# yjcaimeow/pointnerf

Measured on AMD Instinct MI355X. Metric: Mray-samples/sec at 800x800, K=8, 2M neural points; PSNR delta vs ref, higher is better.
Workload: dtype fp32h2

## Files before the change

### pointnerf_amd/csrc/aggregate_x3.hip

```cpp
#include "agg_common.h"


namespace pnr {
namespace {

constexpr int kXT = 64;
constexpr int kXTS = kXT / kKN;
constexpr int kHidPlane = 32 * 64 * 16;
constexpr int kHidTile = 2 * kHidPlane;
constexpr int kXG = 34;
constexpr int kPG = 8;
constexpr int kPlaneX = kXG * kXT * 16;
constexpr int kPlaneP = kPG * kXT * 16;
constexpr int kP1Pitch = kHid + 4;

template <bool H>
struct XL {
  static constexpr int NPL = H ? 2 : 3;
  static constexpr int NPW = H ? 2 : 3;
  static constexpr unsigned kOne = H ? 0x3C00u : 0x3F80u;
  static constexpr int OffPE = NPL * kPlaneX;
  static constexpr int OffEx = OffPE + NPL * kPlaneP;
  static constexpr int NWB = H ? 3 : 2;
  static constexpr int OffWt = OffEx + 2 * 8 * kXT * 4;
  static constexpr int OffPr = OffWt + NWB * kXT * 4;
  static constexpr int OffSf = OffPr + 2 * kXT * 4;
  static constexpr int OffAp = OffSf + NWB * kXTS * 4;
  static constexpr int OffWa = OffAp + 4 * kXT * 4;
  static constexpr int OffH4 = OffWa + kHid * 4;
  static constexpr int OffTq = OffH4 + (H ? kXT * kP1Pitch * 4 : 0);
  static constexpr size_t Lds = (size_t)OffTq + 16;
  static_assert(OffSf % 16 == 0 && OffWa % 16 == 0 && OffH4 % 16 == 0, "16-B aligned LDS arrays");
  static_assert(kXT * kP1Pitch * 4 <= NPL * kPlaneX, "parked P1 fits the layer-input area");
  static_assert(Lds <= 160 * 1024, "LDS budget");
};

constexpr int kProducerPrio = 3;
constexpr int kStoreWindowPrio = 0;

typedef float f32x2n __attribute__((ext_vector_type(2)));
typedef float f32x4n __attribute__((ext_vector_type(4)));

struct X3Args {
  pnr_points pts;
  pnr_samples s;
  pnr_mlp w;
  SplitW wx;
  const float* p1;
  float* hid;
  int32_t* vmask;
  float* out_feat;
  float* out_weight;
  float* out_conf;
  int32_t* tile_ctr;
  pnr_agg_saved sv;
};

__device__ __forceinline__ bool xcd_mode(int64_t nt) { return nt >= 2 * (int64_t)gridDim.x + 16; }
__device__ __forceinline__ int64_t xcd_lo(int64_t nt, int x) { return nt * x / 8; }
__device__ __forceinline__ int64_t xcd_nb(int x) { return ((int)gridDim.x - x + 7) / 8; }

__device__ __forceinline__ int64_t first_tile(int64_t nt) {
  if (!xcd_mode(nt)) return blockIdx.x;
  return xcd_lo(nt, blockIdx.x & 7) + (blockIdx.x >> 3);
}

__device__ __forceinline__ int64_t take_tile(const X3Args& A, int64_t nt) {
  if (!xcd_mode(nt)) return (int64_t)gridDim.x + atomicAdd(A.tile_ctr, 1);
  const int x0 = blockIdx.x & 7;
  for (int i = 0; i < 8; ++i) {
    const int x = (x0 + i) & 7;
    const int64_t t = xcd_lo(nt, x) + xcd_nb(x) + atomicAdd(A.tile_ctr + x, 1);
    if (t < xcd_lo(nt, x + 1)) return t;
  }
  return nt;
}

__device__ __forceinline__ __amdgpu_buffer_rsrc_t rsrc(const void* base) {
  return __builtin_amdgcn_make_buffer_rsrc(const_cast<void*>(base), 0, 0x7fffffff, 0x00020000);
}

template <bool H, int NTK = 8>
__device__ __forceinline__ void load_w(uint4 (&a)[2][XL<H>::NPW], __amdgpu_buffer_rsrc_t rs, int voff, int t) {
  constexpr int NPW = XL<H>::NPW;
#pragma unroll
  for (int T = 0; T < 2; ++T)
#pragma unroll
    for (int pl = 0; pl < NPW; ++pl)
      a[T][pl] = __builtin_bit_cast(
          uint4, __builtin_amdgcn_raw_buffer_load_b128(
                     rs, voff + pl * 1024, (t * NTK + T) * NPW * 1024, 0));
}

template <bool H>
struct WRing {
  static constexpr int kWD = 3;
  uint4 a[kWD][2][XL<H>::NPW];
};

template <bool H, int NTK = 8>
__device__ __forceinline__ void prime(WRing<H>& w, __amdgpu_buffer_rsrc_t rs, int voff) {
#pragma unroll
  for (int d = 0; d < WRing<H>::kWD; ++d) load_w<H, NTK>(w.a[d], rs, voff, d);
}

template <bool H, int NTK = 8, bool ACC2 = false, bool ZACC = false>
__device__ __forceinline__ void layer(f32x16 (&acc)[4], f32x16 (&corr)[4], WRing<H>& w, __amdgpu_buffer_rsrc_t rs,
                                      int voff, const char* planes, int pstride, int nsteps, int lane) {
  static_assert(ACC2 || !ZACC, "zero-start accumulators: with two accumulator sets only");
  static_assert(H || !ACC2, "two accumulator sets: the f16 split only");
  constexpr int NPL = XL<H>::NPL, NPW = XL<H>::NPW, kWD = WRing<H>::kWD;
  const int c = lane & 31, h = lane >> 5;
  const char* base = planes + (h * kXT + c) * 16;
  auto ldb = [&](int t, int pt, uint4 (&bb)[NPL]) {
#pragma unroll
    for (int pl = 0; pl < NPL; ++pl)
      bb[pl] = *reinterpret_cast<const uint4*>(base + pl * pstride + (2 * t * kXT + 32 * pt) * 16);
// ... 146 lines not shown
          lrelu_splith(v[0], v[1], k, ks, a0, a1);
          lrelu_splith(v[2], v[3], k, ks, b0, b1);
          char* d = planes + ((4 * (T0 + T) + q) * kXT + 32 * pt + c) * 16 + 8 * h;
          *reinterpret_cast<uint2*>(d) = make_uint2(a0, b0);
          *reinterpret_cast<uint2*>(d + pstride) = make_uint2(a1, b1);
        }
    return;
  }
#pragma unroll
  for (int pt = 0; pt < 2; ++pt)
#pragma unroll
    for (int T = 0; T < 2; ++T)
#pragma unroll
      for (int q = 0; q < 4; ++q) {
        const f32x16& v = acc[2 * pt + T];
        unsigned a0, a1, a2, b0, b1, b2;
        split2(fmaxf(v[4 * q], s * v[4 * q]), fmaxf(v[4 * q + 1], s * v[4 * q + 1]), a0, a1, a2);
        split2(fmaxf(v[4 * q + 2], s * v[4 * q + 2]), fmaxf(v[4 * q + 3], s * v[4 * q + 3]), b0, b1, b2);
        char* d = planes + ((4 * (T0 + T) + q) * kXT + 32 * pt + c) * 16 + 8 * h;
        *reinterpret_cast<uint2*>(d) = make_uint2(a0, b0);
        *reinterpret_cast<uint2*>(d + kPlaneX) = make_uint2(a1, b1);
        *reinterpret_cast<uint2*>(d + 2 * kPlaneX) = make_uint2(a2, b2);
      }
}

template <bool H>
__device__ __forceinline__ void store_act(const f32x16 (&acc)[4], char* planes, float s, float mul, int lane,
                                          int T0, int pstride = kPlaneX) {
  store_act<H, false>(acc, acc, planes, s, mul, lane, T0, pstride);
}

template <bool H>
__device__ __forceinline__ void acc_init(f32x16 (&acc)[4], const float* bias, float inv_scale, int lane, int T0) {
  if constexpr (H) {
    const int h = lane >> 5;
#pragma unroll
    for (int T = 0; T < 2; ++T)
#pragma unroll
      for (int q = 0; q < 4; ++q) {
        const float4 b = *reinterpret_cast<const float4*>(bias + 32 * (T0 + T) + 8 * q + 4 * h);
        const float v[4] = {b.x * inv_scale, b.y * inv_scale, b.z * inv_scale, b.w * inv_scale};
#pragma unroll
        for (int i = 0; i < 4; ++i) {
          acc[T][4 * q + i] = v[i];
          acc[2 + T][4 * q + i] = v[i];
        }
      }
  } else {
#pragma unroll
    for (int i = 0; i < 4; ++i) acc[i] = (f32x16){0.f};
  }
}
constexpr int kBiasSteps(bool H) { return H ? 16 : 17; }

template <bool H>
__device__ __forceinline__ void store_group(char* planes, int pstride, int g, int pair, const float (&v)[8]) {
  if constexpr (H) {
    uint4 p0, p1;
    splith(v[0], v[1], p0.x, p1.x);
    splith(v[2], v[3], p0.y, p1.y);
    splith(v[4], v[5], p0.z, p1.z);
    splith(v[6], v[7], p0.w, p1.w);
    char* d = planes + (g * kXT + pair) * 16;
    *reinterpret_cast<uint4*>(d) = p0;
    *reinterpret_cast<uint4*>(d + pstride) = p1;
    return;
  }
  uint4 p0, p1, p2;
  split2(v[0], v[1], p0.x, p1.x, p2.x);
  split2(v[2], v[3], p0.y, p1.y, p2.y);
  split2(v[4], v[5], p0.z, p1.z, p2.z);
  split2(v[6], v[7], p0.w, p1.w, p2.w);
  char* d = planes + (g * kXT + pair) * 16;
  *reinterpret_cast<uint4*>(d) = p0;
  *reinterpret_cast<uint4*>(d + pstride) = p1;
  *reinterpret_cast<uint4*>(d + 2 * pstride) = p2;
}

struct GatherState {
  int64_t tile;
  int64_t row;
  int pid;
  float sw[3], sp[3];
  int64_t dmap;
  bool active;
};

__device__ __forceinline__ void gather_row(const X3Args& A, int64_t tile, int lane, GatherState& g) {
  const int64_t v = tile * kXTS + (lane >> 3);
  g.tile = tile;
  g.active = v < eff_n(A.s);
  g.row = g.active ? sample_row(A.s, v) : 0;
}

__device__ __forceinline__ void gather_sample(const X3Args& A, int lane, GatherState& g) {
  const int k = lane & 7, K = A.s.K;
  g.pid = (g.active && k < K) ? A.s.pidx[g.row * K + k] : -1;
#pragma unroll
  for (int a = 0; a < 3; ++a) {
    g.sw[a] = g.active ? A.s.sample_w[g.row * 3 + a] : 0.f;
    g.sp[a] = g.active ? A.s.sample_p[g.row * 3 + a] : 0.f;
  }
  g.dmap = A.s.dir_map ? (int64_t)A.s.dir_map[g.row] : g.row;
}

template <bool H, bool TR = false>
__device__ __forceinline__ void gather(const X3Args& A, const GatherState& g, int nb, int nw, char* lds, int pw, int lane,
                                       float (&dr6)[6]) {
  using L = XL<H>;
  float Rw[9];
#pragma unroll
  for (int i = 0; i < 9; ++i) Rw[i] = A.w.rw2c ? A.w.rw2c[i] : (i % 4 == 0 ? 1.f : 0.f);
  float cam_c[3] = {0.f, 0.f, 0.f}, cam_R[9] = {1.f, 0.f, 0.f, 0.f, 1.f, 0.f, 0.f, 0.f, 1.f};
  if (!A.pts.pers) {
#pragma unroll
    for (int i = 0; i < 3; ++i) cam_c[i] = A.pts.campos[i];
#pragma unroll
    for (int i = 0; i < 9; ++i) cam_R[i] = A.pts.camrot[i];
  }
  const int j = lane >> 3, k = lane & 7;
  const int K = A.s.K;
  const bool active = g.active;
  const int64_t row = g.row;
  const bool valid = g.pid >= 0;
  const int64_t prow = valid ? g.pid : (active && k < K ? 0 : -1);
  float sw[3], sp[3], vd[3] = {0.f, 0.f, 0.f};
#pragma unroll
  for (int a = 0; a < 3; ++a) {
    sw[a] = g.sw[a];
    sp[a] = g.sp[a];
  }
  const int64_t drow = active ? g.dmap / A.s.dir_div : 0;
  if (active && pw == 0) {
#pragma unroll
    for (int a = 0; a < 3; ++a) vd[a] = A.s.dirs[drow * 3 + a];
  }
  float pw3[3] = {0.f, 0.f, 0.f}, pp[3] = {0.f, 0.f, 0.f}, col[3] = {0.f, 0.f, 0.f}, pdir[3] = {0.f, 0.f, 0.f};
  float cf = 1.f;
  if (valid) {
#pragma unroll
    for (int a = 0; a < 3; ++a) pw3[a] = A.pts.xyz[prow * 3 + a];
    if (pw == 0) {
#pragma unroll
      for (int a = 0; a < 3; ++a) {
        col[a] = A.pts.color ? A.pts.color[prow * 3 + a] : 0.f;
        pdir[a] = A.pts.dir ? A.pts.dir[prow * 3 + a] : 0.f;
      }
    }
    if (A.pts.pers) {
#pragma unroll
      for (int a = 0; a < 3; ++a) pp[a] = A.pts.pers[prow * 3 + a];
    } else {
      pair_pers(A.pts, A.s, drow, pw3, cam_c, cam_R, pp);
    }
  }
  if (pw == 0 && A.pts.conf && prow >= 0) cf = A.pts.conf[prow];
  float d6[6];
  d6[0] = pw3[0] - sw[0];
  d6[1] = pw3[1] - sw[1];
  d6[2] = pw3[2] - sw[2];
  d6[3] = pp[0] * pp[2] - sp[0] * sp[2];
  d6[4] = pp[1] * pp[2] - sp[1] * sp[2];
  d6[5] = pp[2] - sp[2];
  mat3(Rw, d6, dr6);
  dr6[3] = d6[3];
  dr6[4] = d6[4];
  dr6[5] = d6[5];
  if (A.pts.rw2c) rot_point(A.pts.rw2c, prow, d6, dr6);
  if (pw == 0) {
    const float nrm = sqrtf(d6[0] * d6[0] + d6[1] * d6[1] + d6[2] * d6[2]);
    const float wl = valid ? 1.f / fmaxf(nrm, 1e-6f) : 0.f;
    const float wsum = xor8_sum(wl);
    const float wn = wl / fmaxf(wsum, 1e-8f);
    const float confc = fminf(fmaxf(cf, 1e-4f), 1.f);
    const bool samp_valid = xor8_sum(valid ? 1.f : 0.f) > 0.f;
    float vrot[3], drot[3];
    mat3(Rw, vd, vrot);
    mat3(Rw, pdir, drot);
    if (A.pts.rw2c) {
      rot_point(A.pts.rw2c, prow, pdir, drot);
      rot_point(A.pts.rw2c, active ? slot0_point(A.s, row) : 0, vd, vrot);
    }
    const float dot = drot[0] * vrot[0] + drot[1] * vrot[1] + drot[2] * vrot[2];
    const float ex[8] = {col[0], col[1], col[2], drot[0] - vrot[0], drot[1] - vrot[1], drot[2] - vrot[2], dot, 1.f};
    float* exL = reinterpret_cast<float*>(lds + L::OffEx) + nb * 8 * kXT;
#pragma unroll
    for (int e = 0; e < 8; ++e) exL[e * kXT + lane] = ex[e];
    reinterpret_cast<float*>(lds + L::OffWt)[nw * kXT + lane] = wn * confc;
    reinterpret_cast<int*>(lds + L::OffPr)[nb * kXT + lane] = valid ? (int)prow : -1;
    if (k == 0) reinterpret_cast<int*>(lds + L::OffSf)[nw * kXTS + j] = active && samp_valid;
    if (active && k < K) {
      if (A.out_weight) A.out_weight[row * K + k] = wn;
      if (A.out_conf) A.out_conf[row * K + k] = confc;
    }
    if (TR && active) {
      const int64_t pr = g.tile * kXT + lane;
      float4* x = reinterpret_cast<float4*>(A.sv.x3e + pr * 32);
      x[0] = make_float4(ex[0], ex[1], ex[2], ex[3]);
      x[1] = make_float4(ex[4], ex[5], ex[6], ex[7]);
#pragma unroll
      for (int e = 2; e < 8; ++e) x[e] = make_float4(0.f, 0.f, 0.f, 0.f);
      A.sv.wt[pr] = wn * confc;
      A.sv.wn[pr] = wn;
      A.sv.prow[pr] = valid ? (int32_t)prow : -1;
    }
  }
}

template <bool H>
__device__ __forceinline__ void pe_store(char* lds, int lane, int e, float sn, float cs) {
  using L = XL<H>;
  const int r = 2 * e;
  char* d = lds + L::OffPE + ((r >> 3) * kXT + lane) * 16 + 2 * (r & 7);
  if constexpr (H) {
    unsigned x0, x1;
    splith(sn, cs, x0, x1);
    *reinterpret_cast<unsigned*>(d) = x0;
    *reinterpret_cast<unsigned*>(d + kPlaneP) = x1;
  } else {
    unsigned x0, x1, x2;
    split2(sn, cs, x0, x1, x2);
    *reinterpret_cast<unsigned*>(d) = x0;
    *reinterpret_cast<unsigned*>(d + kPlaneP) = x1;
    *reinterpret_cast<unsigned*>(d + 2 * kPlaneP) = x2;
  }
}

template <bool H, int PART, bool TR = false>
__device__ __forceinline__ void pe_planes(char* lds, int pw, int lane, const float (&dr6)[6],
                                          const X3Args* A = nullptr, const GatherState* g = nullptr) {
  using L = XL<H>;
  float* pe5 = TR && g->active ? A->sv.pe5 + (g->tile * kXT + lane) * 64 : nullptr;
  if (pw == 0 && PART == 0) {
    char* pz = lds + L::OffPE + (7 * kXT + lane) * 16 + 8;
#pragma unroll
    for (int pl = 0; pl < L::NPL; ++pl) *reinterpret_cast<uint2*>(pz + pl * kPlaneP) = make_uint2(0u, 0u);
    if (TR && pe5) *reinterpret_cast<float4*>(pe5 + 60) = make_float4(0.f, 0.f, 0.f, 0.f);
  }
  const int mine = __builtin_amdgcn_readfirstlane(PART == 0 ? pw : 4 + pw);
#pragma unroll
  for (int ch = 4 * PART; ch < (PART == 0 ? 4 : 6); ++ch) {
    if (ch != mine) continue;
    float s0, c0, s1, c1, s2, c2, s3, c3, s4, c4;
    sincosf(dr6[ch], &s0, &c0);
    sincosf(dr6[ch] * 2.f, &s1, &c1);
    sincosf(dr6[ch] * 4.f, &s2, &c2);
    sincosf(dr6[ch] * 8.f, &s3, &c3);
    sincosf(dr6[ch] * 16.f, &s4, &c4);
    pe_store<H>(lds, lane, 5 * ch + 0, s0, c0);
    pe_store<H>(lds, lane, 5 * ch + 1, s1, c1);
    pe_store<H>(lds, lane, 5 * ch + 2, s2, c2);
    pe_store<H>(lds, lane, 5 * ch + 3, s3, c3);
    pe_store<H>(lds, lane, 5 * ch + 4, s4, c4);
    if (TR && pe5) {
      const float sv[10] = {s0, c0, s1, c1, s2, c2, s3, c3, s4, c4};
#pragma unroll
      for (int i = 0; i < 10; i += 2) *reinterpret_cast<float2*>(pe5 + 10 * ch + i) = make_float2(sv[i], sv[i + 1]);
    }
  }
}

#define X3_SYNC() __syncthreads()

template <bool H, bool TR = false>
__device__ __forceinline__ void finalize_alpha(const X3Args& A, char* lds, int buf, int64_t tile, int lane) {
  using L = XL<H>;
// ... 141 lines not shown
        *reinterpret_cast<uint4*>(XP + pl * kPlaneX + (32 * kXT + lane) * 16) =
            make_uint4(pl == 0 ? L::kOne : 0u, 0u, 0u, 0u);
    }
    acc_init<H>(acc, A.w.b4, in2 / sc4, lane, T0);
    X3_SYNC();
    layer<H, 8, A2>(acc, corr, wr, r4, voff, XP, kPlaneX, kBiasSteps(H), lane);
    prime<H>(wr, r1, voff);
    if constexpr (H) {
      if constexpr (TR) save_act_train<H>(A, acc, A.sv.h4, 3, tile, n, neg, lane, T0, sc4);
      float* H4 = reinterpret_cast<float*>(lds + L::OffH4);
#pragma unroll
      for (int pt = 0; pt < 2; ++pt)
#pragma unroll
        for (int T = 0; T < 2; ++T)
#pragma unroll
          for (int q = 0; q < 4; ++q) {
            float v[4];
#pragma unroll
            for (int i = 0; i < 4; ++i)
              v[i] = A2 ? fold2(acc[2 * pt + T][4 * q + i], corr[2 * pt + T][4 * q + i]) : acc[2 * pt + T][4 * q + i];
            *reinterpret_cast<float4*>(H4 + (32 * pt + c) * kP1Pitch + 32 * (T0 + T) + 8 * q + 4 * h) =
                make_float4(v[0], v[1], v[2], v[3]);
          }
    } else {
      if constexpr (TR) save_act_train<H>(A, acc, A.sv.h4, 3, tile, n, neg, lane, T0, 1.f);
      const float* wtL = reinterpret_cast<const float*>(lds + L::OffWt) + buf * kXT;
      const int* sflag = reinterpret_cast<const int*>(lds + L::OffSf) + buf * kXTS;
      float pa_part[2] = {0.f, 0.f};
      const int i8 = c & 7;
      const bool b2 = (i8 & 4) != 0, b1 = (i8 & 2) != 0, b0 = (i8 & 1) != 0;
#pragma unroll
      for (int pt = 0; pt < 2; ++pt) {
        const float wtp = wtL[32 * pt + c];
        const int sj = (32 * pt + c) >> 3;
        const int64_t vo = tile * kXTS + sj;
        const bool wrt = vo < n && sflag[sj];
#pragma unroll
        for (int T = 0; T < 2; ++T) {
          float v[16];
#pragma unroll
          for (int r = 0; r < 16; ++r) {
            const float hv = lrelu(H ? acc[2 * pt + T][r] * sc4 : acc[2 * pt + T][r], neg);
            pa_part[pt] += waL[32 * (T0 + T) + acc_row(r, h)] * hv;
            v[r] = wtp * hv;
          }
          float w8[8], w4[4], w2[2];
#pragma unroll
          for (int q = 0; q < 8; ++q) {
            const float send = b2 ? v[q] : v[q + 8];
            const float recv = __builtin_bit_cast(
                float, __builtin_amdgcn_mov_dpp(__builtin_bit_cast(int, send), 0x141, 0xf, 0xf, false));
            w8[q] = (b2 ? v[q + 8] : v[q]) + recv;
          }
#pragma unroll
          for (int q = 0; q < 4; ++q) {
            const float send = b1 ? w8[q] : w8[q + 4];
            const float recv = __builtin_bit_cast(
                float, __builtin_amdgcn_mov_dpp(__builtin_bit_cast(int, send), 0x4E, 0xf, 0xf, false));
            w4[q] = (b1 ? w8[q + 4] : w8[q]) + recv;
          }
#pragma unroll
          for (int q = 0; q < 2; ++q) {
            const float send = b0 ? w4[q] : w4[q + 2];
            const float recv = __builtin_bit_cast(
                float, __builtin_amdgcn_mov_dpp(__builtin_bit_cast(int, send), 0xB1, 0xf, 0xf, false));
            w2[q] = (b0 ? w4[q + 2] : w4[q]) + recv;
          }
          if (wrt)
            __builtin_nontemporal_store(
                (f32x2n){w2[0], w2[1]},
                reinterpret_cast<f32x2n*>(A.hid + vo * kHid + 32 * (T0 + T) + ((2 * i8) & 3) + 8 * (i8 >> 1) + 4 * h));
        }
        pa_part[pt] += __shfl_xor(pa_part[pt], 32);
      }
      if (h == 0) {
        apart[wid * kXT + c] = pa_part[0];
        apart[wid * kXT + 32 + c] = pa_part[1];
      }
    }
    X3_SYNC();
  }
}

__device__ __forceinline__ unsigned fetch_p1(f32x4n (&r)[16], const X3Args& A, const int* prow, int pw, int lane) {
  int64_t rows[16];
#pragma unroll
  for (int i = 0; i < 16; ++i) {
    const int pr = prow[16 * pw + i];
    rows[i] = pr < 0 ? -1 : (A.pts.used_map ? (int64_t)A.pts.used_map[pr] : (int64_t)pr);
  }
  unsigned empty = 0;
#pragma unroll
  for (int i = 0; i < 16; ++i) {
    r[i] = __builtin_nontemporal_load(reinterpret_cast<const f32x4n*>(A.p1 + (rows[i] < 0 ? 0 : rows[i]) * kHid) +
                                      lane);
    if (rows[i] < 0) empty |= 1u << i;
  }
  return empty;
}

__device__ __forceinline__ void park_p1(const f32x4n (&r)[16], unsigned empty, char* lds, int pw, int lane) {
  float* P1L = reinterpret_cast<float*>(lds);
#pragma unroll
  for (int i = 0; i < 16; ++i) {
    const f32x4n z = {0.f, 0.f, 0.f, 0.f};
    *reinterpret_cast<f32x4n*>(P1L + (16 * pw + i) * kP1Pitch + 4 * lane) = ((empty >> i) & 1) ? z : r[i];
  }
}

struct TailState {
  float hs[8], pa[8];
};

template <int PART, bool TR = false>
__device__ __forceinline__ void producer_tail(const X3Args& A, char* lds, int slot, int64_t tile, int pw, int lane,
                                              TailState& ts, float& chk) {
  using L = XL<true>;
  const int64_t n = eff_n(A.s);
  const int j = 2 * pw + (lane >> 5), ng = lane & 31;
  const float* H4 = reinterpret_cast<const float*>(lds + L::OffH4);
  const float* wtL = reinterpret_cast<const float*>(lds + L::OffWt) + slot * kXT + 8 * j;
  const int sf = reinterpret_cast<const int*>(lds + L::OffSf)[slot * kXTS + j];
  const float* waL = reinterpret_cast<const float*>(lds + L::OffWa) + 8 * ng;
  const float sc = A.wx.scale[3], neg = A.w.neg_slope;
  const float4 wa0 = *reinterpret_cast<const float4*>(waL), wa1 = *reinterpret_cast<const float4*>(waL + 4);
  const float wa[8] = {wa0.x, wa0.y, wa0.z, wa0.w, wa1.x, wa1.y, wa1.z, wa1.w};
  const float4 wt0 = *reinterpret_cast<const float4*>(wtL), wt1 = *reinterpret_cast<const float4*>(wtL + 4);
  const float wt[8] = {wt0.x, wt0.y, wt0.z, wt0.w, wt1.x, wt1.y, wt1.z, wt1.w};
  float (&hs)[8] = ts.hs;
  float (&pa)[8] = ts.pa;
#pragma unroll
  for (int k = 4 * PART; k < 4 * PART + 4; ++k) {
    const float* row = H4 + (8 * j + k) * kP1Pitch + 8 * ng;
    const float4 a = *reinterpret_cast<const float4*>(row), b = *reinterpret_cast<const float4*>(row + 4);
    const float x[8] = {a.x, a.y, a.z, a.w, b.x, b.y, b.z, b.w};
    float p = 0.f;
#pragma unroll
    for (int i = 0; i < 8; ++i) {
      const float hv = lrelu(x[i] * sc, neg);
      p = fmaf(wa[i], hv, p);
      hs[i] = k == 0 ? wt[0] * hv : fmaf(wt[k], hv, hs[i]);
    }
    pa[k] = p;
  }
  if (PART == 0) return;
  const bool b4 = (ng & 16) != 0, b3 = (ng & 8) != 0, b2 = (ng & 4) != 0;
  float r4[4], r2[2];
#pragma unroll
  for (int q = 0; q < 4; ++q) r4[q] = (b4 ? pa[q + 4] : pa[q]) + __shfl_xor(b4 ? pa[q] : pa[q + 4], 16);
#pragma unroll
  for (int q = 0; q < 2; ++q) r2[q] = (b3 ? r4[q + 2] : r4[q]) + __shfl_xor(b3 ? r4[q] : r4[q + 2], 8);
  float r1 = (b2 ? r2[1] : r2[0]) + __shfl_xor(b2 ? r2[0] : r2[1], 4);
  r1 += __shfl_xor(r1, 2);
  r1 += __shfl_xor(r1, 1);
  const float pk = r1 + A.w.ba[0];
  if (TR && (ng & 3) == 0 && tile * kXTS + j < n) A.sv.pa[tile * kXT + 8 * j + (ng >> 2)] = pk;
  const float alpha_k = A.w.act_super ? softplus(pk - 1.f) : fmaxf(pk, 0.f);
  float as = wtL[ng >> 2] * alpha_k;
  as += __shfl_xor(as, 4);
  as += __shfl_xor(as, 8);
  as += __shfl_xor(as, 16);
  chk = fmaf(0.f, (hs[0] + hs[1]) + (hs[2] + hs[3]) + (hs[4] + hs[5]) + (hs[6] + hs[7]) + as, chk);
  const int64_t vo = tile * kXTS + j;
  if (vo < n) {
    if (ng == 0) {
      A.vmask[vo] = sf;
      if (sf) A.out_feat[vo * (kC + 1)] = as;
    }
    if (TR) {
      if (sf) {
        float4* dst = reinterpret_cast<float4*>(A.hid + vo * kHid + 8 * ng);
        dst[0] = make_float4(hs[0], hs[1], hs[2], hs[3]);
        dst[1] = make_float4(hs[4], hs[5], hs[6], hs[7]);
      }
    } else if (sf) {
      typedef unsigned u32x4n __attribute__((ext_vector_type(4)));
      unsigned a[4], b[4];
#pragma unroll
      for (int i = 0; i < 4; ++i) splith(hs[2 * i], hs[2 * i + 1], a[i], b[i]);
      const u32x4n p0 = {a[0], a[1], a[2], a[3]}, p1 = {b[0], b[1], b[2], b[3]};
      u32x4n* dst = reinterpret_cast<u32x4n*>(reinterpret_cast<char*>(A.hid) + (vo / kXT) * kHidTile +
                                              (ng * kXT + vo % kXT) * 16);
      dst[0] = p0;
      dst[kHidPlane / 16] = p1;
    }
  }
}

template <bool H, bool TR = false>
__device__ __forceinline__ void producer_loop(const X3Args& A, char* lds, int pw, int lane) {
  using L = XL<H>;
  constexpr bool SW = H && !TR;
  const int64_t n = eff_n(A.s);
  const int64_t ntiles = cdiv(n, kXTS);
  __builtin_amdgcn_s_setprio(kProducerPrio);
  f32x4n p1r[16];
  unsigned p1e = 0;
  float dr6[6];
  GatherState g;
  gather_row(A, first_tile(ntiles), lane, g);
  gather_sample(A, lane, g);
  gather<H, TR>(A, g, 0, 0, lds, pw, lane, dr6);
  pe_planes<H, 0, TR>(lds, pw, lane, dr6, &A, &g);
  pe_planes<H, 1, TR>(lds, pw, lane, dr6, &A, &g);
  int* TQ = reinterpret_cast<int*>(lds + L::OffTq);
  if (pw == 0 && lane == 0) TQ[1] = (int)take_tile(A, ntiles);
  X3_SYNC();
  p1e = fetch_p1(p1r, A, reinterpret_cast<const int*>(lds + L::OffPr), pw, lane);
  X3_SYNC();
  float chk = 0.f;
  TailState ts;
  int it = 0;
  int64_t prev = -1;
  for (int64_t tile = first_tile(ntiles); tile < ntiles; prev = tile, tile = TQ[(it + 1) & 3], ++it) {
    const int nbuf = (it & 1) ^ 1;
    const int nw = H ? (it + 1) % 3 : nbuf;
    const int64_t next = TQ[(it + 1) & 3];
    if (pw == 0 && lane == 0) TQ[(it + 2) & 3] = next < ntiles ? (int)take_tile(A, ntiles) : (int)ntiles;
    park_p1(p1r, p1e, lds, pw, lane);
    gather_row(A, next, lane, g);
    X3_SYNC();
    if (!H && pw == 0 && it > 0) finalize_alpha<H, TR>(A, lds, nbuf, prev, lane);
    X3_SYNC();
    gather_sample(A, lane, g);
    X3_SYNC();
    gather<H, TR>(A, g, nbuf, nw, lds, pw, lane, dr6);
    if constexpr (H)
      if (it > 0) producer_tail<0, TR>(A, lds, (it + 2) % 3, prev, pw, lane, ts, chk);
    X3_SYNC();
    p1e = fetch_p1(p1r, A, reinterpret_cast<const int*>(lds + L::OffPr) + nbuf * kXT, pw, lane);
    X3_SYNC();
    if constexpr (!SW) pe_planes<H, 0, TR>(lds, pw, lane, dr6, &A, &g);
    if constexpr (H)
      if (it > 0) producer_tail<1, TR>(A, lds, (it + 2) % 3, prev, pw, lane, ts, chk);
    X3_SYNC();
    if constexpr (SW) {
      __builtin_amdgcn_s_setprio(kStoreWindowPrio);
      pe_planes<H, 0, TR>(lds, pw, lane, dr6, &A, &g);
      __builtin_amdgcn_s_setprio(kProducerPrio);
    }
    X3_SYNC();
    pe_planes<H, 1, TR>(lds, pw, lane, dr6, &A, &g);
    X3_SYNC();
  }
  if constexpr (H) {
    if (it > 0) {
      producer_tail<0, TR>(A, lds, (it - 1) % 3, prev, pw, lane, ts, chk);
      producer_tail<1, TR>(A, lds, (it - 1) % 3, prev, pw, lane, ts, chk);
    }
    if (A.wx.range_flag && chk != 0.f) atomicOr(A.wx.range_flag, 1);
  } else {
    if (pw == 0 && it > 0) finalize_alpha<H, TR>(A, lds, (it - 1) & 1, prev, lane);
  }
}

template <bool H, bool TR = false>
__device__ __forceinline__ void pairs_body(const X3Args& A) {
  extern __shared__ __attribute__((aligned(16))) char lds[];
  const int lane = threadIdx.x & 63, wid = threadIdx.x >> 6;
  if (threadIdx.x < kHid) reinterpret_cast<float*>(lds + XL<H>::OffWa)[threadIdx.x] = A.w.wa[threadIdx.x];
  if (wid < 4) {
    X3_SYNC();
    consumer_loop<H, TR>(A, lds, wid, lane);
  } else {
    producer_loop<H, TR>(A, lds, wid - 4, lane);
  }
}

__global__ void __launch_bounds__(512, 1) k_pairs_x3(X3Args A) { pairs_body<false>(A); }
__global__ void __launch_bounds__(512, 1) k_pairs_h2(X3Args A) { pairs_body<true>(A); }
__global__ void __launch_bounds__(512, 1) k_pairs_x3_train(X3Args A) { pairs_body<false, true>(A); }
__global__ void __launch_bounds__(512, 1) k_pairs_h2_train(X3Args A) { pairs_body<true, true>(A); }

constexpr int kCG = 18;
constexpr int kCPlane = kCG * kXT * 16;
constexpr size_t kColH2Lds = 2 * (size_t)kCPlane;
constexpr int kOPitch = kC + 4;
static_assert((size_t)kXT * kOPitch * 4 <= kColH2Lds, "output staging must fit the planes");

struct ColH2Args {
  pnr_samples s;
  pnr_mlp w;
  const void* pack[4];
  float scale[3];
  int32_t* range_flag;
  const float* hid;
  const int32_t* vmask;
  float* out_feat;
  const float* rw2c_pp;
  const float* hid_rows;
  float* vpe;
  float* hc[3];
};

template <int G0, int NG>
__device__ __forceinline__ void color_load_hid(const ColH2Args& A, char* lds, int64_t tile) {
  const int lane = threadIdx.x & 63, pl = threadIdx.x >> 6;
  const char* src = reinterpret_cast<const char*>(A.hid) + tile * kHidTile + lane * 16;
#pragma unroll
  for (int g = 0; g < NG; ++g) {
    __builtin_amdgcn_global_load_lds(
        (const __attribute__((address_space(1))) void*)(src + pl * kHidPlane + (G0 + g) * kXT * 16),
        (__attribute__((address_space(3))) void*)(lds + pl * kCPlane + g * kXT * 16), 16, 0, 0);
  }
}

template <int G0, int NG>
__device__ __forceinline__ void color_split_hid(const ColH2Args& A, char* lds, int64_t tile, int64_t n) {
  const int lane = threadIdx.x & 63, wid = threadIdx.x >> 6;
  const int64_t v = tile * kXT + lane;
  const bool ok = v < n;
  const float4* src = reinterpret_cast<const float4*>(A.hid_rows + (ok ? v : 0) * kHid);
#pragma unroll
  for (int gg = 0; gg < (NG + 1) / 2; ++gg) {
    const int g = 2 * gg + wid;
    if (g >= NG) break;
    const float4 a = ok ? src[2 * (G0 + g)] : make_float4(0.f, 0.f, 0.f, 0.f);
    const float4 b = ok ? src[2 * (G0 + g) + 1] : make_float4(0.f, 0.f, 0.f, 0.f);
    const float g8[8] = {a.x, a.y, a.z, a.w, b.x, b.y, b.z, b.w};
    store_group<true>(lds, kCPlane, g, lane, g8);
  }
}

__device__ __forceinline__ void save_act_rows(const f32x16 (&acc)[4], float* dst, int64_t v0, int64_t n, float neg,
                                              float scale, int lane, int T0) {
  const int c = lane & 31, h = lane >> 5;
#pragma unroll
  for (int pt = 0; pt < 2; ++pt) {
    const int64_t v = v0 + 32 * pt + c;
    if (v >= n) continue;
#pragma unroll
    for (int T = 0; T < 2; ++T)
#pragma unroll
      for (int q = 0; q < 4; ++q) {
        const f32x16& a = acc[2 * pt + T];
        *reinterpret_cast<float4*>(dst + v * kC + 32 * (T0 + T) + 8 * q + 4 * h) =
            make_float4(lrelu(a[4 * q] * scale, neg), lrelu(a[4 * q + 1] * scale, neg),
                        lrelu(a[4 * q + 2] * scale, neg), lrelu(a[4 * q + 3] * scale, neg));
      }
  }
}

template <bool TR>
__global__ void __launch_bounds__(128) __attribute__((amdgpu_waves_per_eu(2, 2))) k_color_h2(ColH2Args A) {
  extern __shared__ __attribute__((aligned(16))) char lds[];
  const int lane = threadIdx.x & 63, wid = threadIdx.x >> 6;
  const int c = lane & 31, h = lane >> 5;
  const int64_t n = eff_n(A.s);
  const int64_t ntiles = cdiv(n, kXT);
  const float neg = A.w.neg_slope;
  float Rw[9];
#pragma unroll
  for (int i = 0; i < 9; ++i) Rw[i] = A.w.rw2c ? A.w.rw2c[i] : (i % 4 == 0 ? 1.f : 0.f);
// ... 220 lines not shown
  return PNR_OK;
}

int launch_color_h2(const pnr_samples& s, const pnr_mlp& w, const void* const pack[4], const float scale[3],
                    int32_t* range_flag, const float* hid, const int32_t* vmask, float* out_feat, hipStream_t st,
                    const float* rw2c_pp, const pnr_agg_saved* train) {
  static bool attr = false;
  if (!attr) {
    PNR_HIP(hipFuncSetAttribute(reinterpret_cast<const void*>(&k_color_h2<false>),
                                hipFuncAttributeMaxDynamicSharedMemorySize, (int)kColH2Lds));
    PNR_HIP(hipFuncSetAttribute(reinterpret_cast<const void*>(&k_color_h2<true>),
                                hipFuncAttributeMaxDynamicSharedMemorySize, (int)kColH2Lds));
    attr = true;
  }
  ColH2Args a;
  a.s = s;
  a.w = w;
  for (int i = 0; i < 4; ++i) a.pack[i] = pack[i];
  for (int i = 0; i < 3; ++i) a.scale[i] = scale[i];
  a.range_flag = range_flag;
  a.hid = hid;
  a.vmask = vmask;
  a.out_feat = out_feat;
  a.rw2c_pp = rw2c_pp;
  a.hid_rows = train ? train->hid : nullptr;
  a.vpe = train ? train->vpe : nullptr;
  a.hc[0] = train ? train->hc1 : nullptr;
  a.hc[1] = train ? train->hc2 : nullptr;
  a.hc[2] = train ? train->hc3 : nullptr;
  const dim3 grid(grid_for(cdiv(s.n_max, kXT), 1, 256 * 4));
  if (train) hipLaunchKernelGGL(k_color_h2<true>, grid, dim3(128), kColH2Lds, st, a);
  else hipLaunchKernelGGL(k_color_h2<false>, grid, dim3(128), kColH2Lds, st, a);
  PNR_LAUNCH_CHECK();
  return PNR_OK;
}

namespace {

__global__ void __launch_bounds__(256) k_hid_rows_h2(float* hid, int64_t tiles) {
  typedef _Float16 h8 __attribute__((ext_vector_type(8)));
  const int s = threadIdx.x & 63, g0 = 8 * (threadIdx.x >> 6);
  for (int64_t tile = blockIdx.x; tile < tiles; tile += gridDim.x) {
    char* base = reinterpret_cast<char*>(hid) + tile * kHidTile;
    uint4 hi[8], lo[8];
#pragma unroll
    for (int g = 0; g < 8; ++g) {
      hi[g] = *reinterpret_cast<const uint4*>(base + ((g0 + g) * kXT + s) * 16);
      lo[g] = *reinterpret_cast<const uint4*>(base + kHidPlane + ((g0 + g) * kXT + s) * 16);
    }
    __syncthreads();
    float* row = hid + (tile * kXT + s) * kHid;
#pragma unroll
    for (int g = 0; g < 8; ++g) {
      const h8 a = __builtin_bit_cast(h8, hi[g]), b = __builtin_bit_cast(h8, lo[g]);
      float x[8];
#pragma unroll
      for (int i = 0; i < 8; ++i) x[i] = fmaf((float)b[i], 1.f / 2048.f, (float)a[i]);
      float4* dst = reinterpret_cast<float4*>(row + 8 * (g0 + g));
      dst[0] = make_float4(x[0], x[1], x[2], x[3]);
      dst[1] = make_float4(x[4], x[5], x[6], x[7]);
    }
    __syncthreads();
  }
}

}

int launch_hid_rows_h2(float* hid, int64_t n_max, hipStream_t st) {
  const int64_t tiles = cdiv(n_max, kXT);
  hipLaunchKernelGGL(k_hid_rows_h2, dim3(grid_for(tiles, 1, 256 * 8)), dim3(256), 0, st, hid, tiles);
  PNR_LAUNCH_CHECK();
  return PNR_OK;
}

template <bool H>
int launch_pairs_split(const pnr_points& pts, const pnr_samples& s, const pnr_mlp& w, const SplitW& wx,
                       const float* p1, float* hid, int32_t* vmask, float* out_feat, float* out_weight,
                       float* out_conf, int32_t* tile_ctr, hipStream_t st, const pnr_agg_saved* sv) {
  const void* fn = H ? (sv ? reinterpret_cast<const void*>(&k_pairs_h2_train) : reinterpret_cast<const void*>(&k_pairs_h2))
                     : (sv ? reinterpret_cast<const void*>(&k_pairs_x3_train) : reinterpret_cast<const void*>(&k_pairs_x3));
  static bool attr[2] = {false, false};
  if (!attr[sv ? 1 : 0]) {
    PNR_HIP(hipFuncSetAttribute(fn, hipFuncAttributeMaxDynamicSharedMemorySize, (int)XL<H>::Lds));
    attr[sv ? 1 : 0] = true;
  }
  X3Args a;
  a.pts = pts;
  a.s = s;
  a.w = w;
  a.wx = wx;
  a.p1 = p1;
  a.hid = hid;
  a.vmask = vmask;
  a.out_feat = out_feat;
  a.out_weight = out_weight;
  a.out_conf = out_conf;
  a.tile_ctr = tile_ctr;
  if (sv) a.sv = *sv;
  else memset(&a.sv, 0, sizeof(a.sv));
  PNR_HIP(hipMemsetAsync(tile_ctr, 0, 8 * sizeof(int32_t), st));
  const int64_t tiles = cdiv(s.n_max, kXTS);
  if (H && sv)
    hipLaunchKernelGGL(k_pairs_h2_train, dim3(grid_for(tiles, 1, 256)), dim3(512), XL<H>::Lds, st, a);
  else if (H)
    hipLaunchKernelGGL(k_pairs_h2, dim3(grid_for(tiles, 1, 256)), dim3(512), XL<H>::Lds, st, a);
  else if (sv)
    hipLaunchKernelGGL(k_pairs_x3_train, dim3(grid_for(tiles, 1, 256)), dim3(512), XL<H>::Lds, st, a);
  else
    hipLaunchKernelGGL(k_pairs_x3, dim3(grid_for(tiles, 1, 256)), dim3(512), XL<H>::Lds, st, a);
  PNR_LAUNCH_CHECK();
  return PNR_OK;
}
template int launch_pairs_split<false>(const pnr_points&, const pnr_samples&, const pnr_mlp&, const SplitW&,
                                       const float*, float*, int32_t*, float*, float*, float*, int32_t*,
                                       hipStream_t, const pnr_agg_saved*);
template int launch_pairs_split<true>(const pnr_points&, const pnr_samples&, const pnr_mlp&, const SplitW&,
                                      const float*, float*, int32_t*, float*, float*, float*, int32_t*,
                                      hipStream_t, const pnr_agg_saved*);

}
```

Baseline: 826.9.

## Add specialised h2 render kernel with LDS-cached constants and uniform P1 fetch

Adds a k_pairs_h2_rs kernel, chosen at launch when the inputs match the common render configuration (no pers, no rw2c, color/dir/conf present, no weight outputs). In that kernel, camera and rotation constants, the alpha bias and the effective sample count are staged once in LDS. Optional-pointer branches are compiled out, and per-sample products are precomputed. fetch_p1 reads point rows with a vectorised LDS load and readfirstlane so the row address is wave-uniform. The aim is to cut scalar/global constant reloads and branching in the producer warps, at the cost of an extra kernel variant and slightly different FMA rounding, which can move PSNR.

```diff
diff --git a/pointnerf_amd/csrc/aggregate_x3.hip b/pointnerf_amd/csrc/aggregate_x3.hip
--- a/pointnerf_amd/csrc/aggregate_x3.hip
+++ b/pointnerf_amd/csrc/aggregate_x3.hip
@@ -1,3 +1,5 @@
+#include <cstdlib>
+
 #include "agg_common.h"
 
 
@@ -30,9 +32,11 @@
   static constexpr int OffH4 = OffWa + kHid * 4;
   static constexpr int OffTq = OffH4 + (H ? kXT * kP1Pitch * 4 : 0);
   static constexpr size_t Lds = (size_t)OffTq + 16;
+  static constexpr int OffCs = OffTq + 16;
+  static constexpr size_t LdsRS = (size_t)OffCs + 96;
   static_assert(OffSf % 16 == 0 && OffWa % 16 == 0 && OffH4 % 16 == 0, "16-B aligned LDS arrays");
   static_assert(kXT * kP1Pitch * 4 <= NPL * kPlaneX, "parked P1 fits the layer-input area");
-  static_assert(Lds <= 160 * 1024, "LDS budget");
+  static_assert(OffCs % 16 == 0 && LdsRS <= 160 * 1024, "LDS budget");
 };
 
 constexpr int kProducerPrio = 3;
@@ -345,17 +349,32 @@
   int64_t row;
   int pid;
   float sw[3], sp[3];
+  float q3, q4;
   int64_t dmap;
   bool active;
 };
 
-__device__ __forceinline__ void gather_row(const X3Args& A, int64_t tile, int lane, GatherState& g) {
+template <bool RS>
+__device__ __forceinline__ int64_t tile_n(const X3Args& A, const char* lds) {
+  if constexpr (RS) return *reinterpret_cast<const int64_t*>(lds + XL<true>::OffCs + 88);
+  else return eff_n(A.s);
+}
+template <bool RS>
+__device__ __forceinline__ float alpha_bias(const X3Args& A, const char* lds) {
+  if constexpr (RS) return reinterpret_cast<const float*>(lds + XL<true>::OffCs)[21];
+  else return A.w.ba[0];
+}
+
+template <bool LC = false>
+__device__ __forceinline__ void gather_row(const X3Args& A, int64_t tile, int lane, GatherState& g,
+                                           const char* lds = nullptr) {
   const int64_t v = tile * kXTS + (lane >> 3);
   g.tile = tile;
-  g.active = v < eff_n(A.s);
+  g.active = v < tile_n<LC>(A, lds);
   g.row = g.active ? sample_row(A.s, v) : 0;
 }
 
+template <bool RS = false>
 __device__ __forceinline__ void gather_sample(const X3Args& A, int lane, GatherState& g) {
   const int k = lane & 7, K = A.s.K;
   g.pid = (g.active && k < K) ? A.s.pidx[g.row * K + k] : -1;
@@ -365,17 +384,47 @@
     g.sp[a] = g.active ? A.s.sample_p[g.row * 3 + a] : 0.f;
   }
   g.dmap = A.s.dir_map ? (int64_t)A.s.dir_map[g.row] : g.row;
-}
-
-template <bool H, bool TR = false>
+  if constexpr (RS) {
+    g.q3 = g.sp[0] * g.sp[2];
+    g.q4 = g.sp[1] * g.sp[2];
+  }
+}
+
+__device__ __forceinline__ float sum012(float a0, float b0, float a1, float b1, float a2, float b2) {
+  return __builtin_fmaf(a2, b2, __builtin_fmaf(a1, b1, a0 * b0));
+}
+__device__ __forceinline__ float sum102(float a0, float b0, float a1, float b1, float a2, float b2) {
+  return __builtin_fmaf(a2, b2, __builtin_fmaf(a0, b0, a1 * b1));
+}
+
+template <bool H, bool TR = false, bool RS = false, bool LC = false>
 __device__ __forceinline__ void gather(const X3Args& A, const GatherState& g, int nb, int nw, char* lds, int pw, int lane,
                                        float (&dr6)[6]) {
   using L = XL<H>;
   float Rw[9];
-#pragma unroll
-  for (int i = 0; i < 9; ++i) Rw[i] = A.w.rw2c ? A.w.rw2c[i] : (i % 4 == 0 ? 1.f : 0.f);
   float cam_c[3] = {0.f, 0.f, 0.f}, cam_R[9] = {1.f, 0.f, 0.f, 0.f, 1.f, 0.f, 0.f, 0.f, 1.f};
-  if (!A.pts.pers) {
+  if constexpr (LC) {
+    const float4* c4 = reinterpret_cast<const float4*>(lds + L::OffCs);
+    float cs[24];
+#pragma unroll
+    for (int q = 0; q < 6; ++q) {
+      const float4 v = c4[q];
+      cs[4 * q] = v.x;
+      cs[4 * q + 1] = v.y;
+      cs[4 * q + 2] = v.z;
+      cs[4 * q + 3] = v.w;
+    }
+#pragma unroll
+    for (int i = 0; i < 9; ++i) Rw[i] = cs[i];
+#pragma unroll
+    for (int i = 0; i < 3; ++i) cam_c[i] = cs[9 + i];
+#pragma unroll
+    for (int i = 0; i < 9; ++i) cam_R[i] = cs[12 + i];
+  } else {
+#pragma unroll
+    for (int i = 0; i < 9; ++i) Rw[i] = A.w.rw2c ? A.w.rw2c[i] : (i % 4 == 0 ? 1.f : 0.f);
+  }
+  if (!LC && !A.pts.pers) {
 #pragma unroll
     for (int i = 0; i < 3; ++i) cam_c[i] = A.pts.campos[i];
 #pragma unroll
@@ -410,7 +459,15 @@
         pdir[a] = A.pts.dir ? A.pts.dir[prow * 3 + a] : 0.f;
       }
     }
-    if (A.pts.pers) {
+    if constexpr (RS) {
+      const float s[3] = {pw3[0] - cam_c[0], pw3[1] - cam_c[1], pw3[2] - cam_c[2]};
+      float xc[3];
+#pragma unroll
+      for (int j = 0; j < 3; ++j) xc[j] = sum102(s[0], cam_R[j], s[1], cam_R[3 + j], s[2], cam_R[6 + j]);
+      pp[0] = __fdiv_rn(xc[0], xc[2]);
+      pp[1] = __fdiv_rn(xc[1], xc[2]);
+      pp[2] = xc[2];
+    } else if (A.pts.pers) {
 #pragma unroll
       for (int a = 0; a < 3; ++a) pp[a] = A.pts.pers[prow * 3 + a];
     } else {
@@ -422,29 +479,49 @@
   d6[0] = pw3[0] - sw[0];
   d6[1] = pw3[1] - sw[1];
   d6[2] = pw3[2] - sw[2];
-  d6[3] = pp[0] * pp[2] - sp[0] * sp[2];
-  d6[4] = pp[1] * pp[2] - sp[1] * sp[2];
+  if constexpr (RS) {
+    d6[3] = __builtin_fmaf(pp[0], pp[2], -g.q3);
+    d6[4] = __builtin_fmaf(pp[1], pp[2], -g.q4);
+  } else {
+    d6[3] = pp[0] * pp[2] - sp[0] * sp[2];
+    d6[4] = pp[1] * pp[2] - sp[1] * sp[2];
+  }
   d6[5] = pp[2] - sp[2];
-  mat3(Rw, d6, dr6);
+  if constexpr (RS) {
+#pragma unroll
+    for (int j = 0; j < 3; ++j) dr6[j] = sum012(d6[0], Rw[3 * j], d6[1], Rw[3 * j + 1], d6[2], Rw[3 * j + 2]);
+  } else {
+    mat3(Rw, d6, dr6);
+  }
   dr6[3] = d6[3];
   dr6[4] = d6[4];
   dr6[5] = d6[5];
   if (A.pts.rw2c) rot_point(A.pts.rw2c, prow, d6, dr6);
   if (pw == 0) {
-    const float nrm = sqrtf(d6[0] * d6[0] + d6[1] * d6[1] + d6[2] * d6[2]);
+    const float nrm = RS ? sqrtf(sum012(d6[0], d6[0], d6[1], d6[1], d6[2], d6[2]))
+                         : sqrtf(d6[0] * d6[0] + d6[1] * d6[1] + d6[2] * d6[2]);
     const float wl = valid ? 1.f / fmaxf(nrm, 1e-6f) : 0.f;
     const float wsum = xor8_sum(wl);
     const float wn = wl / fmaxf(wsum, 1e-8f);
     const float confc = fminf(fmaxf(cf, 1e-4f), 1.f);
     const bool samp_valid = xor8_sum(valid ? 1.f : 0.f) > 0.f;
     float vrot[3], drot[3];
-    mat3(Rw, vd, vrot);
-    mat3(Rw, pdir, drot);
+    if constexpr (RS) {
+#pragma unroll
+      for (int j = 0; j < 3; ++j) {
+        vrot[j] = sum102(vd[0], Rw[3 * j], vd[1], Rw[3 * j + 1], vd[2], Rw[3 * j + 2]);
+        drot[j] = sum102(pdir[0], Rw[3 * j], pdir[1], Rw[3 * j + 1], pdir[2], Rw[3 * j + 2]);
+      }
+    } else {
+      mat3(Rw, vd, vrot);
+      mat3(Rw, pdir, drot);
+    }
     if (A.pts.rw2c) {
       rot_point(A.pts.rw2c, prow, pdir, drot);
       rot_point(A.pts.rw2c, active ? slot0_point(A.s, row) : 0, vd, vrot);
     }
-    const float dot = drot[0] * vrot[0] + drot[1] * vrot[1] + drot[2] * vrot[2];
+    const float dot = RS ? sum012(drot[0], vrot[0], drot[1], vrot[1], drot[2], vrot[2])
+                         : drot[0] * vrot[0] + drot[1] * vrot[1] + drot[2] * vrot[2];
     const float ex[8] = {col[0], col[1], col[2], drot[0] - vrot[0], drot[1] - vrot[1], drot[2] - vrot[2], dot, 1.f};
     float* exL = reinterpret_cast<float*>(lds + L::OffEx) + nb * 8 * kXT;
 #pragma unroll
@@ -752,7 +829,29 @@
   }
 }
 
+template <bool RS = false>
 __device__ __forceinline__ unsigned fetch_p1(f32x4n (&r)[16], const X3Args& A, const int* prow, int pw, int lane) {
+  if constexpr (RS) {
+    const int4* p4 = reinterpret_cast<const int4*>(prow + 16 * pw);
+    int pr[16];
+#pragma unroll
+    for (int q = 0; q < 4; ++q) {
+      const int4 v = p4[q];
+      pr[4 * q] = v.x;
+      pr[4 * q + 1] = v.y;
+      pr[4 * q + 2] = v.z;
+      pr[4 * q + 3] = v.w;
+    }
+    unsigned empty = 0;
+#pragma unroll
+    for (int i = 0; i < 16; ++i) {
+      const int row = __builtin_amdgcn_readfirstlane(pr[i]);
+      r[i] = __builtin_nontemporal_load(reinterpret_cast<const f32x4n*>(A.p1 + (int64_t)(row < 0 ? 0 : row) * kHid) +
+                                        lane);
+      empty |= (row < 0 ? 1u : 0u) << i;
+    }
+    return empty;
+  }
   int64_t rows[16];
 #pragma unroll
   for (int i = 0; i < 16; ++i) {
@@ -782,11 +881,11 @@
   float hs[8], pa[8];
 };
 
-template <int PART, bool TR = false>
+template <int PART, bool TR = false, bool RS = false>
 __device__ __forceinline__ void producer_tail(const X3Args& A, char* lds, int slot, int64_t tile, int pw, int lane,
                                               TailState& ts, float& chk) {
   using L = XL<true>;
-  const int64_t n = eff_n(A.s);
+  const int64_t n = tile_n<RS>(A, lds);
   const int j = 2 * pw + (lane >> 5), ng = lane & 31;
   const float* H4 = reinterpret_cast<const float*>(lds + L::OffH4);
   const float* wtL = reinterpret_cast<const float*>(lds + L::OffWt) + slot * kXT + 8 * j;
@@ -823,7 +922,7 @@
   float r1 = (b2 ? r2[1] : r2[0]) + __shfl_xor(b2 ? r2[0] : r2[1], 4);
   r1 += __shfl_xor(r1, 2);
   r1 += __shfl_xor(r1, 1);
-  const float pk = r1 + A.w.ba[0];
+  const float pk = r1 + alpha_bias<RS>(A, lds);
   if (TR && (ng & 3) == 0 && tile * kXTS + j < n) A.sv.pa[tile * kXT + 8 * j + (ng >> 2)] = pk;
   const float alpha_k = A.w.act_super ? softplus(pk - 1.f) : fmaxf(pk, 0.f);
   float as = wtL[ng >> 2] * alpha_k;
@@ -857,7 +956,7 @@
   }
 }
 
-template <bool H, bool TR = false>
+template <bool H, bool TR = false, bool RS = false>
 __device__ __forceinline__ void producer_loop(const X3Args& A, char* lds, int pw, int lane) {
   using L = XL<H>;
   constexpr bool SW = H && !TR;
@@ -869,14 +968,14 @@
   float dr6[6];
   GatherState g;
   gather_row(A, first_tile(ntiles), lane, g);
-  gather_sample(A, lane, g);
-  gather<H, TR>(A, g, 0, 0, lds, pw, lane, dr6);
+  gather_sample<RS>(A, lane, g);
+  gather<H, TR, RS>(A, g, 0, 0, lds, pw, lane, dr6);
   pe_planes<H, 0, TR>(lds, pw, lane, dr6, &A, &g);
   pe_planes<H, 1, TR>(lds, pw, lane, dr6, &A, &g);
   int* TQ = reinterpret_cast<int*>(lds + L::OffTq);
   if (pw == 0 && lane == 0) TQ[1] = (int)take_tile(A, ntiles);
   X3_SYNC();
-  p1e = fetch_p1(p1r, A, reinterpret_cast<const int*>(lds + L::OffPr), pw, lane);
+  p1e = fetch_p1<RS>(p1r, A, reinterpret_cast<const int*>(lds + L::OffPr), pw, lane);
   X3_SYNC();
   float chk = 0.f;
   TailState ts;
@@ -888,21 +987,21 @@
     const int64_t next = TQ[(it + 1) & 3];
     if (pw == 0 && lane == 0) TQ[(it + 2) & 3] = next < ntiles ? (int)take_tile(A, ntiles) : (int)ntiles;
     park_p1(p1r, p1e, lds, pw, lane);
-    gather_row(A, next, lane, g);
+    gather_row<RS>(A, next, lane, g, lds);
     X3_SYNC();
     if (!H && pw == 0 && it > 0) finalize_alpha<H, TR>(A, lds, nbuf, prev, lane);
     X3_SYNC();
-    gather_sample(A, lane, g);
-    X3_SYNC();
-    gather<H, TR>(A, g, nbuf, nw, lds, pw, lane, dr6);
+    gather_sample<RS>(A, lane, g);
+    X3_SYNC();
+    gather<H, TR, RS, RS>(A, g, nbuf, nw, lds, pw, lane, dr6);
     if constexpr (H)
-      if (it > 0) producer_tail<0, TR>(A, lds, (it + 2) % 3, prev, pw, lane, ts, chk);
-    X3_SYNC();
-    p1e = fetch_p1(p1r, A, reinterpret_cast<const int*>(lds + L::OffPr) + nbuf * kXT, pw, lane);
+      if (it > 0) producer_tail<0, TR, RS>(A, lds, (it + 2) % 3, prev, pw, lane, ts, chk);
+    X3_SYNC();
+    p1e = fetch_p1<RS>(p1r, A, reinterpret_cast<const int*>(lds + L::OffPr) + nbuf * kXT, pw, lane);
     X3_SYNC();
     if constexpr (!SW) pe_planes<H, 0, TR>(lds, pw, lane, dr6, &A, &g);
     if constexpr (H)
-      if (it > 0) producer_tail<1, TR>(A, lds, (it + 2) % 3, prev, pw, lane, ts, chk);
+      if (it > 0) producer_tail<1, TR, RS>(A, lds, (it + 2) % 3, prev, pw, lane, ts, chk);
     X3_SYNC();
     if constexpr (SW) {
       __builtin_amdgcn_s_setprio(kStoreWindowPrio);
@@ -915,8 +1014,8 @@
   }
   if constexpr (H) {
     if (it > 0) {
-      producer_tail<0, TR>(A, lds, (it - 1) % 3, prev, pw, lane, ts, chk);
-      producer_tail<1, TR>(A, lds, (it - 1) % 3, prev, pw, lane, ts, chk);
+      producer_tail<0, TR, RS>(A, lds, (it - 1) % 3, prev, pw, lane, ts, chk);
+      producer_tail<1, TR, RS>(A, lds, (it - 1) % 3, prev, pw, lane, ts, chk);
     }
     if (A.wx.range_flag && chk != 0.f) atomicOr(A.wx.range_flag, 1);
   } else {
@@ -924,21 +1023,49 @@
   }
 }
 
-template <bool H, bool TR = false>
+template <bool H, bool TR = false, bool RS = false>
 __device__ __forceinline__ void pairs_body(const X3Args& A) {
+  static_assert(!RS || (H && !TR), "render specialisation: the h2 inference kernel only");
   extern __shared__ __attribute__((aligned(16))) char lds[];
   const int lane = threadIdx.x & 63, wid = threadIdx.x >> 6;
   if (threadIdx.x < kHid) reinterpret_cast<float*>(lds + XL<H>::OffWa)[threadIdx.x] = A.w.wa[threadIdx.x];
+  if constexpr (RS) {
+    if (wid == 4) {
+      float* cs = reinterpret_cast<float*>(lds + XL<H>::OffCs);
+      if (lane < 9) cs[lane] = A.w.rw2c ? A.w.rw2c[lane] : (lane % 4 == 0 ? 1.f : 0.f);
+      else if (lane < 12) cs[lane] = A.pts.campos[lane - 9];
+      else if (lane < 21) cs[lane] = A.pts.camrot[lane - 12];
+      else if (lane == 21) cs[21] = A.w.ba[0];
+      else if (lane == 22) *reinterpret_cast<int64_t*>(cs + 22) = eff_n(A.s);
+    }
+  }
   if (wid < 4) {
     X3_SYNC();
     consumer_loop<H, TR>(A, lds, wid, lane);
   } else {
-    producer_loop<H, TR>(A, lds, wid - 4, lane);
-  }
+    producer_loop<H, TR, RS>(A, lds, wid - 4, lane);
+  }
+}
+
+inline bool render_route(const X3Args& a) {
+  return !a.pts.pers && !a.pts.used_map && !a.pts.rw2c && a.pts.color && a.pts.dir && a.pts.conf &&
+         a.s.dir_map && !a.s.ray_cam && !a.out_weight && !a.out_conf;
 }
 
 __global__ void __launch_bounds__(512, 1) k_pairs_x3(X3Args A) { pairs_body<false>(A); }
 __global__ void __launch_bounds__(512, 1) k_pairs_h2(X3Args A) { pairs_body<true>(A); }
+__global__ void __launch_bounds__(512, 1) k_pairs_h2_rs(X3Args A0) {
+  X3Args A = A0;
+  A.pts.pers = nullptr;
+  A.pts.used_map = nullptr;
+  A.pts.rw2c = nullptr;
+  A.s.ray_cam = nullptr;
+  A.out_weight = nullptr;
+  A.out_conf = nullptr;
+  __builtin_assume(A.pts.color != nullptr && A.pts.dir != nullptr && A.pts.conf != nullptr);
+  __builtin_assume(A.s.dir_map != nullptr);
+  pairs_body<true, false, true>(A);
+}
 __global__ void __launch_bounds__(512, 1) k_pairs_x3_train(X3Args A) { pairs_body<false, true>(A); }
 __global__ void __launch_bounds__(512, 1) k_pairs_h2_train(X3Args A) { pairs_body<true, true>(A); }
 
@@ -1325,6 +1452,9 @@
   static bool attr[2] = {false, false};
   if (!attr[sv ? 1 : 0]) {
     PNR_HIP(hipFuncSetAttribute(fn, hipFuncAttributeMaxDynamicSharedMemorySize, (int)XL<H>::Lds));
+    if (H && !sv)
+      PNR_HIP(hipFuncSetAttribute(reinterpret_cast<const void*>(&k_pairs_h2_rs),
+                                  hipFuncAttributeMaxDynamicSharedMemorySize, (int)XL<true>::LdsRS));
     attr[sv ? 1 : 0] = true;
   }
   X3Args a;
@@ -1345,6 +1475,8 @@
   const int64_t tiles = cdiv(s.n_max, kXTS);
   if (H && sv)
     hipLaunchKernelGGL(k_pairs_h2_train, dim3(grid_for(tiles, 1, 256)), dim3(512), XL<H>::Lds, st, a);
+  else if (H && render_route(a) && !getenv("PNR_H2_GENERAL"))
+    hipLaunchKernelGGL(k_pairs_h2_rs, dim3(grid_for(tiles, 1, 256)), dim3(512), XL<true>::LdsRS, st, a);
   else if (H)
     hipLaunchKernelGGL(k_pairs_h2, dim3(grid_for(tiles, 1, 256)), dim3(512), XL<H>::Lds, st, a);
   else if (sv)
```

New measurement: 841.7 (median of 6 runs). 1.02x the previous value.
